# sa2shun/adaptive-speculative-decoding

Hardware: AMD Instinct MI355X
Metric: verified_tokens_per_s (higher is better)
Workload: dtype bf16; 1 GPU; c3: BASELINE headline: batch 32, draft_len 8, vocab 152064 (Qwen2.5), bf16 logits; step = asd_verify_accept_fused_ex: ONE launch (verify + accept + in-kernel stats->MLP->Bayes->DP epilogue); batch_per_gpu=32, draft_len=8, vocab=152064, accumulate=f32 (epilogue f64), rotating_buffers=9, launch_mode=graph, steps_per_graph=2, settle=6000 untimed steps before the 5 warm-up steps (clock / power-state ramp), tiers=7B-draft / 32B / 72B-target shapes (vocab 152064); logits synthetic, parallelism=single GPU

## Files before the change

### adaptive-speculative-decoding_amd/csrc/predictor_device.hpp

```cpp
#pragma once

#include "decision_device.hpp"
#include "lse_device.hpp"

#include <math.h>

#ifndef ASD_EPI_STAMP
#define ASD_EPI_STAMP(slot) do { } while (0)
#endif

namespace asd {

static __device__ double np_sum_leaf(const double* a, int n) {
    if (n < 8) {
        double res = 0.0;
        for (int i = 0; i < n; ++i) res = res + a[i];
        return res;
    }
    double r[8];
#pragma unroll
    for (int j = 0; j < 8; ++j) r[j] = a[j];
    int i = 8;
    for (; i < n - (n % 8); i += 8) {
#pragma unroll
// ... 286 lines not shown
}
__device__ __forceinline__ void decide_and_store_small(const FusedParams& p, int b, float sc, const DecidePrefetch& d) {
    if (p.score) p.score[b] = sc;
    double prob = static_cast<double>(sc);
    if (p.risk) prob = bayes_adjust1(prob, p.n_obs, p.alpha, p.beta);
    if (p.p_hist) {
        p.p_hist[static_cast<int64_t>(b) * p.L + p.stage_idx] = prob;
        if (p.k_star || p.stop) {
            const int n_dp = p.prefix ? p.stage_idx + 1 : p.L;
            double pp[kDecidePrefetch], cc[kDecidePrefetch], J[kDecidePrefetch + 1];
#pragma unroll
            for (int i = 0; i < kDecidePrefetch; ++i) {
                pp[i] = (i == p.stage_idx) ? prob : d.ph[i];
                cc[i] = d.cc[i];
            }
            int ks;
            static_assert(kDecidePrefetch == 4, "the depth switch below lists 1 ... 4");
            (void)J;
            switch (n_dp) {
                case 1: ks = optimal_stopping_exact<1>(pp, cc, p.lam); break;
                case 2: ks = optimal_stopping_exact<2>(pp, cc, p.lam); break;
                case 3: ks = optimal_stopping_exact<3>(pp, cc, p.lam); break;
                default: ks = optimal_stopping_exact<4>(pp, cc, p.lam); break;
            }
            if (p.k_star) p.k_star[b] = ks;
            if (p.stop) p.stop[b] = (ks == p.stage_idx) ? 1 : 0;
        }
    }
    if (p.theta && p.thr_stop) {
        const double q = static_cast<double>(sc);
        p.thr_stop[b] = (q >= d.theta || p.stage_idx == p.L - 1) ? 1 : 0;
    }
}
__device__ __forceinline__ void decide_and_store(const FusedParams& p, int b, float sc) {
    DecidePrefetch none;
    decide_and_store_impl<false>(p, b, sc, none);
}

struct EpiPrefetch {
    float w[32];
    float wd[ASD_NUM_LP_STATS];
    float b1, w2, b2, xv;
    DecidePrefetch d;
};

__device__ __forceinline__ void epi_prefetch(const FusedParams& p, int b, int lane, EpiPrefetch& e) {
    e.xv = p.feat[static_cast<int64_t>(b) * p.ldf + lane];
    const int j = lane & 31, half = lane >> 5;
#pragma unroll
    for (int i = 0; i < 32; ++i) e.w[i] = p.packed[(half * 32 + i) * 32 + j];
#pragma unroll
    for (int d = 0; d < ASD_NUM_LP_STATS; ++d) e.wd[d] = p.stats_col >= 0 ? p.packed[(p.stats_col + d) * 32 + j] : 0.0f;
    e.b1 = p.packed[64 * 32 + j];
    e.w2 = p.packed[64 * 32 + 32 + j];
    e.b2 = p.packed[64 * 32 + 64];
    if (lane == 0) decide_prefetch(p, b, e.d);
}

__device__ __forceinline__ float epi_phase_a_input(const FusedParams& p, int lane, float xv) {
    const int si = lane - p.stats_col;
    return (p.stats_col >= 0 && si >= 0 && si < ASD_NUM_LP_STATS) ? 0.0f : xv;
}
__device__ __forceinline__ float add_halves(float h) {
    const auto r = __builtin_amdgcn_permlane32_swap(__float_as_uint(h), __float_as_uint(h), false, false);
    return __uint_as_float(r[0]) + __uint_as_float(r[1]);
}
template <typename WD>
__device__ __forceinline__ float epi_score(const FusedParams& p, int lane, float h, const WD& wd, const double (&st)[5], bool overlay,
                                           float b1, float w2, float b2) {
    const int half = lane >> 5;
    if (overlay) {
#pragma unroll
        for (int d = 0; d < ASD_NUM_LP_STATS; ++d) {
            const float sd = (half == ((p.stats_col + d) >> 5)) ? static_cast<float>(st[d]) : 0.0f;
            h = fmaf(wd(d), sd, h);
        }
    }
    h = add_halves(h);
    h = fmaxf(h + b1, 0.0f);
    const float z = wave_sum(half == 0 ? w2 * h : 0.0f);
    ASD_EPI_STAMP(10);
    const float e = __builtin_amdgcn_exp2f(-(z + b2) * kLog2e);
    return __builtin_amdgcn_rcpf(1.0f + e);
}

__device__ __forceinline__ void epi_finish(const FusedParams& p, int b, int lane, float lpv, int n, bool want_stats,
                                           const EpiPrefetch& e, double* dvals, float* xs) {
    xs[lane] = epi_phase_a_input(p, lane, e.xv);
    __builtin_amdgcn_fence(__ATOMIC_RELEASE, "wavefront");
    __builtin_amdgcn_wave_barrier();
    __builtin_amdgcn_fence(__ATOMIC_ACQUIRE, "wavefront");
    const int half = lane >> 5;
    float h = 0.0f;
#pragma unroll
    for (int i = 0; i < 32; ++i) h = fmaf(e.w[i], xs[half * 32 + i], h);
    double st[5] = {0.0, 0.0, 0.0, 0.0, 0.0};
    if (want_stats) {
        wave_logprob_stats_regs(lpv, n, lane, st);
        if (p.stats && lane == 0) {
#pragma unroll
            for (int i = 0; i < 5; ++i) p.stats[5 * static_cast<int64_t>(b) + i] = st[i];
        }
    }
    const float sc = epi_score(p, lane, h, [&](int d) { return e.wd[d]; }, st, want_stats && p.stats_col >= 0, e.b1, e.w2, e.b2);
    if (lane == 0) decide_and_store_impl<true>(p, b, sc, e.d);
}


constexpr int kEpiInKernelMaxK = 16;
constexpr int kEpiDecideLds = 12;
__device__ __forceinline__ void epi_decide_dma(const FusedParams& p, int b, int lane, double* dl) {
    typedef __attribute__((address_space(3))) void lds_void;
    typedef const __attribute__((address_space(1))) void glb_void;
    const int n_dp = p.prefix ? p.stage_idx + 1 : p.L;
    if (p.p_hist && (p.k_star || p.stop) && lane < 2 * n_dp) {
        __builtin_amdgcn_global_load_lds((glb_void*)(reinterpret_cast<const char*>(p.p_hist + static_cast<int64_t>(b) * p.L) + lane * 4),
                                         (lds_void*)reinterpret_cast<char*>(dl), 4, 0, 0);
        __builtin_amdgcn_global_load_lds((glb_void*)(reinterpret_cast<const char*>(p.C) + lane * 4),
                                         (lds_void*)(reinterpret_cast<char*>(dl) + 32), 4, 0, 0);
    }
    if (p.theta && p.thr_stop && lane < 2)
        __builtin_amdgcn_global_load_lds((glb_void*)(reinterpret_cast<const char*>(p.theta + p.stage_idx) + lane * 4),
                                         (lds_void*)(reinterpret_cast<char*>(dl) + 64), 4, 0, 0);
}
__device__ __forceinline__ void epi_decide_from_lds(const double* dl, DecidePrefetch& d) {
#pragma unroll
    for (int i = 0; i < kDecidePrefetch; ++i) {
        d.ph[i] = dl[i];
        d.cc[i] = dl[kDecidePrefetch + i];
    }
    d.theta = dl[2 * kDecidePrefetch];
}

struct EpiPhaseA {
    float h, wd[ASD_NUM_LP_STATS], b1, w2, b2;
};
__device__ __forceinline__ void epi_phase_a_lds(const FusedParams& p, int lane, float xv, const float* wl, float* xs, EpiPhaseA& a) {
    xs[lane] = epi_phase_a_input(p, lane, xv);
    __builtin_amdgcn_fence(__ATOMIC_RELEASE, "wavefront");
    __builtin_amdgcn_wave_barrier();
    __builtin_amdgcn_fence(__ATOMIC_ACQUIRE, "wavefront");
    const int j = lane & 31, half = lane >> 5;
    const int col = p.stats_col >= 0 ? p.stats_col : 0;
#pragma unroll
    for (int d = 0; d < ASD_NUM_LP_STATS; ++d) a.wd[d] = wl[(col + d) * 32 + j];
    a.b1 = wl[64 * 32 + j];
    a.w2 = wl[64 * 32 + 32 + j];
    a.b2 = wl[64 * 32 + 64];
    float h = 0.0f;
#pragma unroll
    for (int i = 0; i < 32; ++i) h = fmaf(wl[(half * 32 + i) * 32 + j], xs[half * 32 + i], h);
    a.h = h;
}
__device__ __forceinline__ void epi_finish_lds(const FusedParams& p, int b, int lane, float lpv, int n, bool want_stats,
                                               const double* decide_lds, const EpiPhaseA& a) {
    double st[5] = {0.0, 0.0, 0.0, 0.0, 0.0};
    if (want_stats) {
        wave_logprob_stats_row16(lpv, n, lane, st);
        if (p.stats && lane == 0) {
#pragma unroll
            for (int i = 0; i < 5; ++i) p.stats[5 * static_cast<int64_t>(b) + i] = st[i];
        }
    }
    ASD_EPI_STAMP(9);
    const float sc = epi_score(p, lane, a.h, [&](int d) { return a.wd[d]; }, st, want_stats && p.stats_col >= 0, a.b1, a.w2, a.b2);
    ASD_EPI_STAMP(11);
    if (lane == 0) {
        DecidePrefetch d;
        epi_decide_from_lds(decide_lds, d);
        decide_and_store_small(p, b, sc, d);
    }
}

constexpr int kEpi2In = 256, kEpi2Hid = 128, kEpi2Waves = 8, kEpi2Cols = kEpi2In / kEpi2Waves;
__device__ __forceinline__ void epi2_partial(const float* packed, int w, int lane, float xv, float& h0, float& h1) {
    h0 = 0.0f;
    h1 = 0.0f;
    const float* wp = packed + static_cast<int64_t>(w) * kEpi2Cols * kEpi2Hid + lane;
#pragma unroll 8
    for (int i = 0; i < kEpi2Cols; ++i) {
        const float x = __uint_as_float(__builtin_amdgcn_readlane(__float_as_uint(xv), i));
        h0 = fmaf(wp[i * kEpi2Hid], x, h0);
        h1 = fmaf(wp[i * kEpi2Hid + 64], x, h1);
    }
}
__device__ __forceinline__ float epi2_feature(const float* feat_row, int stats_col, int w, int lane) {
    const int c = w * kEpi2Cols + (lane & 31);
    const float x = feat_row[c];
    const int si = c - stats_col;
    return (stats_col >= 0 && si >= 0 && si < ASD_NUM_LP_STATS) ? 0.0f : x;
}
struct Epi2Tail {
    float wd0[ASD_NUM_LP_STATS], wd1[ASD_NUM_LP_STATS], b1a, b1b, w2a, w2b, b2;
};
__device__ __forceinline__ void epi2_tail_prefetch(const float* packed, int stats_col, int lane, Epi2Tail& t) {
    const int col = stats_col >= 0 ? stats_col : 0;
#pragma unroll
    for (int d = 0; d < ASD_NUM_LP_STATS; ++d) {
        t.wd0[d] = packed[(col + d) * kEpi2Hid + lane];
        t.wd1[d] = packed[(col + d) * kEpi2Hid + 64 + lane];
    }
    const float* b1 = packed + kEpi2In * kEpi2Hid;
    t.b1a = b1[lane]; t.b1b = b1[64 + lane];
    t.w2a = b1[kEpi2Hid + lane]; t.w2b = b1[kEpi2Hid + 64 + lane];
    t.b2 = b1[2 * kEpi2Hid];
}
__device__ __forceinline__ float epi2_score(const float* part, int lane, const Epi2Tail& t, const double (&st)[5], bool overlay) {
    float h0 = part[lane], h1 = part[64 + lane];
#pragma unroll
    for (int w = 1; w < kEpi2Waves; ++w) {
        h0 = h0 + part[w * kEpi2Hid + lane];
        h1 = h1 + part[w * kEpi2Hid + 64 + lane];
    }
    if (overlay) {
#pragma unroll
        for (int d = 0; d < ASD_NUM_LP_STATS; ++d) {
            const float sd = static_cast<float>(st[d]);
            h0 = fmaf(t.wd0[d], sd, h0);
            h1 = fmaf(t.wd1[d], sd, h1);
        }
    }
    h0 = fmaxf(h0 + t.b1a, 0.0f);
    h1 = fmaxf(h1 + t.b1b, 0.0f);
    const float z = wave_sum(fmaf(t.w2b, h1, t.w2a * h0));
    const float e = __builtin_amdgcn_exp2f(-(z + t.b2) * kLog2e);
    return __builtin_amdgcn_rcpf(1.0f + e);
}
__device__ __forceinline__ void epi2_finish_lds(const FusedParams& p, int b, int lane, float lpv, int n, bool want_stats,
                                                const double* decide_lds, const float* part, const Epi2Tail& t) {
    double st[5] = {0.0, 0.0, 0.0, 0.0, 0.0};
    if (want_stats) {
        wave_logprob_stats_row16(lpv, n, lane, st);
        if (p.stats && lane == 0) {
#pragma unroll
            for (int i = 0; i < 5; ++i) p.stats[5 * static_cast<int64_t>(b) + i] = st[i];
        }
    }
    const float sc = epi2_score(part, lane, t, st, want_stats && p.stats_col >= 0);
    if (lane == 0) {
        DecidePrefetch d;
        epi_decide_from_lds(decide_lds, d);
        decide_and_store_small(p, b, sc, d);
    }
}

}
```

### adaptive-speculative-decoding_amd/csrc/verify_accept.hip

```cpp

#include <hip/hip_runtime.h>

#ifdef ASD_STAMP
__device__ unsigned long long* g_asd_stamps = nullptr;
#define ASD_STAMP_AT(slot)                                                                       \
    do {                                                                                         \
        if (threadIdx.x == 0 && g_asd_stamps)                                                    \
            g_asd_stamps[static_cast<size_t>(blockIdx.y * gridDim.x + blockIdx.x) * 16 + (slot)] = __builtin_amdgcn_s_memrealtime(); \
    } while (0)
#define ASD_EPI_STAMP(slot) ASD_STAMP_AT(slot)
#else
#define ASD_STAMP_AT(slot) do { } while (0)
#endif

#define ASD_DPP_ASM_REDUCTIONS 1
#include "lse_device.hpp"
#include "predictor_device.hpp"

namespace asd {
namespace {

constexpr int kMaxStage = 1024;
constexpr int kTicketStride = 160;
constexpr int kLpLineOffset = 32;
constexpr int kSpinLimit = 1 << 20;
constexpr int kFastMaxK = 32;

struct VerifyParams {
    const void* logits;
    int64_t ld_row;
    const int32_t* tok;
    const float* lp_d;
    const float* u;
    int B, K, V, S;
    int64_t v_offset;
    float* lp_t;
    uint8_t* accept;
    int32_t* n_acc;
    uint64_t* bits;
    float* msg;
    uint32_t* tickets;
    uint64_t* granules;
    uint32_t region;
    float scale2;
    int mode;
    float* row_max_lp;
    float* row_entropy;
    int fused;
    int withhold1;
    FusedParams epi;
};

__device__ __forceinline__ uint64_t poll_slot(uint64_t* slot) {
    uint64_t v = __hip_atomic_load(slot, __ATOMIC_RELAXED, __HIP_MEMORY_SCOPE_AGENT);
    for (int spins = 0; v == 0ull && spins < kSpinLimit; ++spins) {
        __builtin_amdgcn_s_sleep(1);
        v = __hip_atomic_load(slot, __ATOMIC_RELAXED, __HIP_MEMORY_SCOPE_AGENT);
    }
    return v;
}

__device__ __forceinline__ uint64_t poll_more(uint64_t* slot, uint64_t v) {
    for (int spins = 0; v == 0ull && spins < kSpinLimit; ++spins) {
        __builtin_amdgcn_s_sleep(1);
        v = __hip_atomic_load(slot, __ATOMIC_RELAXED, __HIP_MEMORY_SCOPE_AGENT);
    }
    return v;
}

__device__ __forceinline__ void report_lost(uint32_t* workspace_words) {
    __hip_atomic_fetch_or(workspace_words, static_cast<uint32_t>(ASD_WS_LOST_HANDOFF), __ATOMIC_RELAXED, __HIP_MEMORY_SCOPE_AGENT);
}

__device__ __forceinline__ void epi_poison(const FusedParams& e, int b) {
    if (e.score) e.score[b] = NAN;
    if (e.k_star) e.k_star[b] = e.L - 1;
    if (e.stop) e.stop[b] = 0;
    if (e.thr_stop) e.thr_stop[b] = 0;
    if (e.stats) {
        for (int i = 0; i < ASD_NUM_LP_STATS; ++i) e.stats[ASD_NUM_LP_STATS * static_cast<int64_t>(b) + i] = NAN;
    }
}

constexpr int kKernargParamsOffset = 48;
static_assert(alignof(VerifyParams) == 8, "kKernargParamsOffset assumes an 8-byte aligned parameter struct");
#define ASD_PIN(x) asm volatile("" : "+s"(x))
template <typename T>
__device__ __forceinline__ T* pin_global_ptr(T* p) {
    uint64_t bits = reinterpret_cast<uint64_t>(p);
    asm volatile("" : "+s"(bits));
    return (T*)(__attribute__((address_space(1))) T*)bits;
}
#define ASD_PIN_PTR(x) do { x = pin_global_ptr(x); } while (0)
__device__ __forceinline__ void pin_epilogue_params(FusedParams& e) {
    ASD_PIN(e.K); ASD_PIN_PTR(e.feat); ASD_PIN(e.ldf); ASD_PIN(e.stats_col); ASD_PIN_PTR(e.packed);
    ASD_PIN(e.risk); ASD_PIN(e.n_obs); ASD_PIN(e.alpha); ASD_PIN(e.beta);
    ASD_PIN_PTR(e.p_hist); ASD_PIN_PTR(e.C); ASD_PIN(e.lam); ASD_PIN(e.L); ASD_PIN(e.stage_idx); ASD_PIN(e.prefix);
    ASD_PIN_PTR(e.theta); ASD_PIN_PTR(e.score); ASD_PIN_PTR(e.k_star); ASD_PIN_PTR(e.stop); ASD_PIN_PTR(e.thr_stop); ASD_PIN_PTR(e.stats);
}

template <int DT, int UNROLL, bool CHECK, bool STATS>
__device__ __forceinline__ void consume(const u32x4 (&r)[UNROLL], uint32_t off, uint32_t end, float c2, float& m2, float& s,
                                        float& t) {
    using E = Elem<DT>;
#pragma unroll
    for (int j = 0; j < UNROLL; ++j) {
        u32x4 v = r[j];
        if (CHECK) {
            const bool ok = off + static_cast<uint32_t>(j) * 1024u < end;
            const u32x4 neg = {E::kNegInfWord, E::kNegInfWord, E::kNegInfWord, E::kNegInfWord};
            v = ok ? v : neg;
        }
        if (STATS) E::accum3(v, c2, m2, s, t);
        else E::accum(v, c2, m2, s);
    }
}

__device__ __forceinline__ float row_max_logprob(float s) {
    return s > 0.0f ? static_cast<float>(-kLn2d * log2_split(s)) : NAN;
}
__device__ __forceinline__ float row_entropy_nats(float m2, float s, float t, float c2) {
    if (!(s > 0.0f)) return NAN;
    const double L = static_cast<double>(m2) + log2_split(s);
    return static_cast<float>(kLn2d * (L - static_cast<double>(c2) * static_cast<double>(t) / static_cast<double>(s)));
}

template <int DT, int THREADS, int UNROLL, bool NT, bool FUSED, bool STATS = false, int EPI = 1>
__global__ __launch_bounds__(THREADS) void k_verify(const void* a_logits, const int32_t* a_tok, int64_t a_ld_row, int a_V,
                                                    int a_K, int a_S, float a_scale2, int a_own, const VerifyParams p) {
    using E = Elem<DT>;
    constexpr int kWaves = THREADS / 64;
    __shared__ uint32_t next_tile;
    __shared__ __attribute__((aligned(16))) uint64_t stage[kMaxStage];
    __shared__ float stage_t[STATS ? kMaxStage : 1];
    static_assert(EPI == 1 || (EPI == 2 && THREADS == 64 * kEpi2Waves), "the 256 x 128 epilogue is cut over eight waves");
    __shared__ __attribute__((aligned(16))) float wlds[FUSED ? (EPI == 2 ? kEpi2Waves * kEpi2Hid : 64 * 32 + 68) : 4];
    __shared__ __attribute__((aligned(16))) double dlds[FUSED ? kEpiDecideLds : 1];

    ASD_STAMP_AT(0);
#ifdef ASD_STAMP
    if (threadIdx.x == 0 && g_asd_stamps)
        g_asd_stamps[static_cast<size_t>(blockIdx.y * gridDim.x + blockIdx.x) * 16 + 6] = __builtin_amdgcn_s_getreg((31 << 11) | 20) & 0xf;
#endif
    const int tid = threadIdx.x;
    const int lane = tid & 63;
    const int wave = tid >> 6;
    const int S = a_S;
    const float c2 = a_scale2;
    const int row = static_cast<int>(blockIdx.x);
    const int split = static_cast<int>(blockIdx.y);

    const char* rowp = static_cast<const char*>(a_logits) + static_cast<int64_t>(row) * a_ld_row * E::kBytes;
    const uint32_t mis = static_cast<uint32_t>(reinterpret_cast<uintptr_t>(rowp) & 15u);
    int head = mis ? static_cast<int>((16u - mis) / E::kBytes) : 0;
    if (head > a_V) head = a_V;
    const int nvec = (a_V - head) / E::kPerVec;
    const int tail = a_V - head - nvec * E::kPerVec;
    const char* body = rowp + static_cast<int64_t>(head) * E::kBytes;
    int v0 = 0, v1 = nvec;
    if (S > 1) {
        v0 = static_cast<int>(static_cast<uint32_t>(nvec) * static_cast<uint32_t>(split) / static_cast<uint32_t>(S));
        v1 = static_cast<int>(static_cast<uint32_t>(nvec) * static_cast<uint32_t>(split + 1) / static_cast<uint32_t>(S));
    }

    const bool own_row = a_own != 0;
    float x_tok = -INFINITY, lpd = 0.0f, uu = 1.0f;
    uint32_t raw_tok = 0, raw_lpd = 0, raw_u = 0x3f800000u, raw_x = 0;
    bool have_x = false;
    double lu_row = 0.0;
    int vrow = row;
    asm volatile("" : "+v"(vrow));
    const bool gather = own_row || split == 0;
    if (gather && tid == 0) raw_tok = static_cast<uint32_t>(a_tok[vrow]);

    constexpr uint32_t kTileBytes = static_cast<uint32_t>(UNROLL) * 1024u;
    const uint32_t end = v1 > v0 ? static_cast<uint32_t>(v1 - v0) * 16u : 0u;
    const uint32_t n_tiles = (end + kTileBytes - 1) / kTileBytes;
    const uint32_t n_full = end / kTileBytes;
    const __amdgpu_buffer_rsrc_t rsrc = __builtin_amdgcn_make_buffer_rsrc(
        const_cast<char*>(body) + static_cast<int64_t>(v0) * 16, 0, static_cast<int>(end), 0x00020000);
    const uint32_t lane_off = static_cast<uint32_t>(lane) * 16u;
    if (tid == 0) next_tile = 2u * kWaves;
    uint32_t ta = static_cast<uint32_t>(wave), tb = static_cast<uint32_t>(wave) + kWaves;
    u32x4 ra[UNROLL], rb[UNROLL];
#pragma unroll
    for (int j = 0; j < UNROLL; ++j) ra[j] = load16<NT>(rsrc, ta * kTileBytes + static_cast<uint32_t>(j) * 1024u + lane_off);
#pragma unroll
    for (int j = 0; j < UNROLL; ++j) rb[j] = load16<NT>(rsrc, tb * kTileBytes + static_cast<uint32_t>(j) * 1024u + lane_off);
    ASD_STAMP_AT(7);
    __syncthreads();

    asm volatile("" : "+v"(raw_tok));
    const int64_t t_tok = static_cast<int64_t>(static_cast<int32_t>(raw_tok)) - p.v_offset;
    if (gather && tid == 0 && t_tok >= 0 && t_tok < a_V) {
        raw_x = E::raw(rowp, t_tok);
        have_x = true;
    }
    if (own_row && tid == 0 && p.mode == 0) {
        raw_lpd = reinterpret_cast<const uint32_t*>(p.lp_d)[vrow];
        raw_u = reinterpret_cast<const uint32_t*>(p.u)[vrow];
    }
    uint32_t raw_head = 0, raw_tail = 0, raw_feat = 0;
    const bool do_head = wave == 0 && split == 0 && lane < head;
    const bool do_tail = wave == 0 && split == S - 1 && lane >= 32 && lane - 32 < tail;
    if (do_head) raw_head = E::raw(rowp, lane);
    if (do_tail) raw_tail = E::raw(rowp, static_cast<int64_t>(head) + static_cast<int64_t>(nvec) * E::kPerVec + (lane - 32));
    const int b = static_cast<int>(static_cast<uint32_t>(row) / static_cast<uint32_t>(a_K));
    const int k = row - b * a_K;
    const bool fused = FUSED && p.mode == 0;
#define ASD_CLAIM(dst)                                                                                   \
    do {                                                                                                 \
        uint32_t c_ = 0;                                                                                 \
        if (lane == 0) c_ = __hip_atomic_fetch_add(&next_tile, 1u, __ATOMIC_RELAXED, __HIP_MEMORY_SCOPE_WORKGROUP); \
        dst = __builtin_amdgcn_readfirstlane(c_);                                                        \
    } while (0)
#define ASD_REDUCE_TILE(reg, t)                                                                          \
    do {                                                                                                 \
        float tm_ = kSentinel, ts_ = 0.0f, tt_ = 0.0f;                                                   \
        if ((t) < n_full) consume<DT, UNROLL, false, STATS>(reg, (t) * kTileBytes + lane_off, end, c2, tm_, ts_, tt_);   \
        else consume<DT, UNROLL, true, STATS>(reg, (t) * kTileBytes + lane_off, end, c2, tm_, ts_, tt_);                 \
        if (STATS) wave_merge3(tm_, ts_, tt_);                                                           \
        else wave_merge(tm_, ts_);                                                                       \
        if (lane == 0) {                                                                                 \
            stage[(t)] = (static_cast<uint64_t>(__float_as_uint(ts_)) << 32) | __float_as_uint(tm_);     \
            if (STATS) stage_t[(t)] = tt_;                                                               \
        }                                                                                                \
    } while (0)

    bool first = true;
    while (ta < n_tiles) {
        uint32_t tn;
        ASD_CLAIM(tn);
        ASD_REDUCE_TILE(ra, ta);
        if (first) { ASD_STAMP_AT(1); first = false; }
        ta = tn;
#if defined(ASD_LAB) && ASD_LAB == 10
#pragma unroll
        for (int j = 0; j < UNROLL; ++j) asm volatile("" : "+v"(ra[j]));
#else
#pragma unroll
        for (int j = 0; j < UNROLL; ++j) ra[j] = load16<NT>(rsrc, ta * kTileBytes + static_cast<uint32_t>(j) * 1024u + lane_off);
#endif
        if (tb >= n_tiles) break;
        ASD_CLAIM(tn);
        ASD_REDUCE_TILE(rb, tb);
        tb = tn;
#if defined(ASD_LAB) && ASD_LAB == 10
#pragma unroll
        for (int j = 0; j < UNROLL; ++j) asm volatile("" : "+v"(rb[j]));
#else
#pragma unroll
        for (int j = 0; j < UNROLL; ++j) rb[j] = load16<NT>(rsrc, tb * kTileBytes + static_cast<uint32_t>(j) * 1024u + lane_off);
#endif
    }
#undef ASD_CLAIM
#undef ASD_REDUCE_TILE

    ASD_STAMP_AT(2);
#ifdef ASD_STAMP
    if (lane == 0 && g_asd_stamps)
        g_asd_stamps[static_cast<size_t>(gridDim.x * gridDim.y) * 16 + static_cast<size_t>(blockIdx.y * gridDim.x + blockIdx.x) * 16 + wave] = __builtin_amdgcn_s_memrealtime();
#endif
#if defined(ASD_LAB) && (ASD_LAB == 8 || ASD_LAB == 10)
    if (lane == 0 && stage[0] == 0x1234567812345678ull) p.lp_t[row] = 0.0f;
    return;
#endif
    FusedParams ep;
    const int wave_u = __builtin_amdgcn_readfirstlane(wave);
    const bool fin_wg = FUSED && fused && k == a_K - 1 && (own_row || split == S - 1);
    float xv2 = 0.0f;
    const float* packed2 = nullptr;
    int col2 = -1;
    if constexpr (FUSED && EPI == 2) {
        if (fin_wg) {
            typedef const __attribute__((address_space(4))) char* ka_ptr2;
            typedef const __attribute__((address_space(4))) FusedParams* ka_epi_ptr2;
            ka_ptr2 ka2 = (ka_ptr2)__builtin_amdgcn_kernarg_segment_ptr();
            asm volatile("" : "+s"(ka2));
            const ka_epi_ptr2 kp2 = (ka_epi_ptr2)(ka2 + kKernargParamsOffset + __builtin_offsetof(VerifyParams, epi));
            const float* feat2 = pin_global_ptr(kp2->feat);
            int64_t ldf2 = kp2->ldf;
            col2 = kp2->stats_col;
            packed2 = pin_global_ptr(kp2->packed);
            ASD_PIN(ldf2); ASD_PIN(col2);
            xv2 = epi2_feature(feat2 + static_cast<int64_t>(b) * ldf2, col2, wave_u, lane);
        }
    }
    if (wave_u == 0) {
        asm volatile("" : "+v"(raw_x), "+v"(raw_head), "+v"(raw_tail), "+v"(raw_lpd), "+v"(raw_u));
        if (FUSED) {
            typedef const __attribute__((address_space(4))) char* ka_ptr;
            typedef const __attribute__((address_space(4))) FusedParams* ka_epi_ptr;
            ka_ptr ka = (ka_ptr)__builtin_amdgcn_kernarg_segment_ptr();
            asm volatile("" : "+s"(ka));
            const ka_epi_ptr kp = (ka_epi_ptr)(ka + kKernargParamsOffset + __builtin_offsetof(VerifyParams, epi));
            ep.lp = nullptr; ep.ld_lp = 0; ep.n_valid = nullptr; ep.in_dim = 64; ep.hidden = 32; ep.use_lds = 0; ep.B = 0;
            ep.K = kp->K; ep.feat = kp->feat; ep.ldf = kp->ldf; ep.stats_col = kp->stats_col; ep.packed = kp->packed;
            ep.risk = kp->risk; ep.n_obs = kp->n_obs; ep.alpha = kp->alpha; ep.beta = kp->beta;
            ep.p_hist = kp->p_hist; ep.C = kp->C; ep.lam = kp->lam; ep.L = kp->L; ep.stage_idx = kp->stage_idx; ep.prefix = kp->prefix;
            ep.theta = kp->theta; ep.score = kp->score; ep.k_star = kp->k_star; ep.stop = kp->stop; ep.thr_stop = kp->thr_stop;
            ep.stats = kp->stats;
            pin_epilogue_params(ep);
#if defined(ASD_LAB) && ASD_LAB == 5
            if (false) {
#else
            if (EPI == 1 && fin_wg) {
#endif
                typedef __attribute__((address_space(3))) void lds_void;
                typedef const __attribute__((address_space(1))) void glb_void;
                const char* src = reinterpret_cast<const char*>(ep.packed);
#pragma unroll
                for (int ps = 0; ps < 8; ++ps)
                    __builtin_amdgcn_global_load_lds((glb_void*)(src + ps * 1024 + lane * 16), (lds_void*)(reinterpret_cast<char*>(wlds) + ps * 1024), 16, 0, 0);
                __builtin_amdgcn_global_load_lds((glb_void*)(src + 8192 + lane * 4), (lds_void*)(reinterpret_cast<char*>(wlds) + 8192), 4, 0, 0);
                if (lane == 0)
                    __builtin_amdgcn_global_load_lds((glb_void*)(src + 8192 + 256), (lds_void*)(reinterpret_cast<char*>(wlds) + 8192 + 256), 4, 0, 0);
                raw_feat = reinterpret_cast<const uint32_t*>(ep.feat)[static_cast<int64_t>(b) * ep.ldf + lane];
            }
        }
        float hm = kSentinel, hs = 0.0f, ht = 0.0f;
        if (do_head) {
            const float xv = E::from_raw(raw_head);
            accum_scalar(xv, c2, hm, hs);
            if (STATS) ht = hs > 0.0f ? hs * xv : 0.0f;
        }
        if (do_tail) {
            const float xv = E::from_raw(raw_tail);
            accum_scalar(xv, c2, hm, hs);
            if (STATS) ht = hs > 0.0f ? hs * xv : 0.0f;
        }
        if (STATS) wave_merge3(hm, hs, ht);
        else wave_merge(hm, hs);
        if (lane == 0) {
            stage[n_tiles] = (static_cast<uint64_t>(__float_as_uint(hs)) << 32) | __float_as_uint(hm);
            if (STATS) stage_t[n_tiles] = ht;
        }
        if (gather && tid == 0) {
            if (have_x) x_tok = E::from_raw(raw_x);
            if (own_row && p.mode == 0) {
                lpd = __uint_as_float(raw_lpd);
                uu = __uint_as_float(raw_u);
                lu_row = log_u(uu);
            }
        }
    }
    __syncthreads();
    if (wave_u != 0) {
        if constexpr (FUSED && EPI == 2) {
            if (fin_wg) {
                float h0, h1;
                epi2_partial(packed2, wave_u, lane, xv2, h0, h1);
                wlds[wave_u * kEpi2Hid + lane] = h0;
                wlds[wave_u * kEpi2Hid + 64 + lane] = h1;
                __syncthreads();
            }
        }
        return;
    }
    float m2 = kSentinel, s = 0.0f, tsum = 0.0f;
    for (uint32_t t = static_cast<uint32_t>(lane); t <= n_tiles; t += 64) {
        const uint64_t g = stage[t];
        if (STATS) ms_merge3(m2, s, tsum, __uint_as_float(static_cast<uint32_t>(g)), __uint_as_float(static_cast<uint32_t>(g >> 32)), stage_t[t]);
        else ms_merge(m2, s, __uint_as_float(static_cast<uint32_t>(g)), __uint_as_float(static_cast<uint32_t>(g >> 32)));
    }
    if (STATS) wave_merge3(m2, s, tsum);
    else wave_merge(m2, s);
    __builtin_amdgcn_fence(__ATOMIC_RELEASE, "wavefront");
    __builtin_amdgcn_wave_barrier();
    ASD_STAMP_AT(3);

    if (own_row) {
        if (!(FUSED && fused) && lane != 0) return;
        if (p.mode == 1) {
            p.msg[3 * row + 0] = m2;
            p.msg[3 * row + 1] = s;
            p.msg[3 * row + 2] = x_tok;
            return;
        }
        uint32_t* line = p.tickets + static_cast<int64_t>(b) * kTicketStride;
        if (FUSED && fused) {
            float lp = 0.0f;
            bool flag = false;
            if (lane == 0) flag = finish_row(m2, s, x_tok, c2, lpd, lu_row, lp);
            uint64_t* slots = reinterpret_cast<uint64_t*>(line + kLpLineOffset);
            const uint64_t mine = (1ull << 63) | (static_cast<uint64_t>(flag ? 1u : 0u) << 32) | __float_as_uint(lp);
            if (k != p.K - 1) {
                if (lane == 0) {
                    if (row + 1 != p.withhold1) __hip_atomic_store(slots + k, mine, __ATOMIC_RELAXED, __HIP_MEMORY_SCOPE_AGENT);
                    p.lp_t[row] = lp;
                    p.accept[row] = flag ? 1 : 0;
                    if (p.row_max_lp) p.row_max_lp[row] = row_max_logprob(s);
                }
                return;
            }
            ASD_STAMP_AT(4);
            uint64_t sv = __shfl(mine, 0, 64);
            EpiPhaseA pa{};
            Epi2Tail tail2{};
            if constexpr (EPI == 1) {
                asm volatile("s_waitcnt vmcnt(0)" : "+v"(raw_feat) :: "memory");
                if (lane < p.K - 1) sv = __hip_atomic_load(slots + lane, __ATOMIC_RELAXED, __HIP_MEMORY_SCOPE_AGENT);
                epi_phase_a_lds(ep, lane, __uint_as_float(raw_feat), wlds, reinterpret_cast<float*>(stage + 192), pa);
                uint32_t sv_lo = static_cast<uint32_t>(sv), sv_hi = static_cast<uint32_t>(sv >> 32);
                asm volatile("" : "+v"(pa.h), "+v"(pa.wd[0]), "+v"(pa.wd[1]), "+v"(pa.wd[2]), "+v"(pa.wd[3]), "+v"(pa.wd[4]), "+v"(pa.b1), "+v"(pa.w2),
                             "+v"(pa.b2), "+v"(sv_lo), "+v"(sv_hi));
                sv = (static_cast<uint64_t>(sv_hi) << 32) | sv_lo;
            } else {
                if (lane < p.K - 1) sv = __hip_atomic_load(slots + lane, __ATOMIC_RELAXED, __HIP_MEMORY_SCOPE_AGENT);
                epi2_tail_prefetch(packed2, col2, lane, tail2);
                float h0, h1;
                epi2_partial(packed2, 0, lane, xv2, h0, h1);
                wlds[lane] = h0;
                wlds[64 + lane] = h1;
                __syncthreads();
                uint32_t sv_lo = static_cast<uint32_t>(sv), sv_hi = static_cast<uint32_t>(sv >> 32);
                asm volatile("" : "+v"(sv_lo), "+v"(sv_hi));
                sv = (static_cast<uint64_t>(sv_hi) << 32) | sv_lo;
            }
            epi_decide_dma(ep, b, lane, dlds);
            if (lane == 0) {
                p.lp_t[row] = lp;
                p.accept[row] = flag ? 1 : 0;
                if (p.row_max_lp) p.row_max_lp[row] = row_max_logprob(s);
            }
#if defined(ASD_LAB) && (ASD_LAB == 2 || ASD_LAB == 5)
            sv = __shfl(mine, 0, 64);
            if (lane < p.K - 1) __hip_atomic_store(slots + lane, 0ull, __ATOMIC_RELAXED, __HIP_MEMORY_SCOPE_AGENT);
#else
            if (lane < p.K - 1) {
                sv = poll_more(slots + lane, sv);
                __hip_atomic_store(slots + lane, 0ull, __ATOMIC_RELAXED, __HIP_MEMORY_SCOPE_AGENT);
            }
#endif
            const bool lost = lane < p.K && sv == 0ull;
            const unsigned long long bal = __ballot(lane < p.K && ((sv >> 32) & 1ull));
            if (lane == 0) {
                const unsigned long long inv = ~bal;
                const int n = inv ? __builtin_ctzll(inv) : 64;
                p.n_acc[b] = n < p.K ? n : p.K;
                if (p.bits) p.bits[b] = bal;
            }
            ASD_STAMP_AT(5);
            if (__ballot(lost) != 0ull) {
                if (lane == 0) {
                    epi_poison(ep, b);
                    report_lost(p.tickets);
                }
                return;
            }
#if defined(ASD_LAB) && (ASD_LAB == 1 || ASD_LAB == 2 || ASD_LAB == 5)
            if (lane == 0 && ep.score) ep.score[b] = pa.h + pa.wd[0] + pa.b1 + pa.w2 + pa.b2 + __uint_as_float(static_cast<uint32_t>(sv));
            return;
#endif
            if constexpr (EPI == 1)
                epi_finish_lds(ep, b, lane, __uint_as_float(static_cast<uint32_t>(sv)), p.K, ep.stats_col >= 0 || ep.stats != nullptr, dlds, pa);
            else
                epi2_finish_lds(ep, b, lane, __uint_as_float(static_cast<uint32_t>(sv)), p.K, ep.stats_col >= 0 || ep.stats != nullptr, dlds, wlds, tail2);
            ASD_STAMP_AT(8);
            return;
        }
        if (lane == 0) {
            float lp;
            const bool flag = finish_row(m2, s, x_tok, c2, lpd, lu_row, lp);
            p.lp_t[row] = lp;
            p.accept[row] = flag ? 1 : 0;
            if (p.row_max_lp) p.row_max_lp[row] = row_max_logprob(s);
            if (STATS) {
                if (p.row_entropy) p.row_entropy[row] = row_entropy_nats(m2, s, tsum, c2);
            }
            uint64_t* word = reinterpret_cast<uint64_t*>(line + 2);
            const uint64_t mine = (1ull << 32) | (static_cast<uint64_t>(flag ? 1u : 0u) << k);
            ASD_STAMP_AT(4);
#if defined(ASD_LAB) && ASD_LAB == 9
            if (mine == 0x1234ull) p.n_acc[b] = 0;
            return;
#endif
            const uint64_t old = __hip_atomic_fetch_add(word, mine, __ATOMIC_RELAXED, __HIP_MEMORY_SCOPE_AGENT);
            if (static_cast<uint32_t>(old >> 32) == static_cast<uint32_t>(p.K - 1)) {
                const uint32_t mask = static_cast<uint32_t>(old | mine);
                const uint32_t inv = ~mask;
                const int n = inv ? __builtin_ctz(inv) : 32;
                p.n_acc[b] = n < p.K ? n : p.K;
                if (p.bits) p.bits[b] = mask;
                __hip_atomic_store(word, 0ull, __ATOMIC_RELAXED, __HIP_MEMORY_SCOPE_AGENT);
            }
#ifdef ASD_STAMP
            asm volatile("s_waitcnt vmcnt(0)" ::: "memory");
            if (g_asd_stamps) g_asd_stamps[static_cast<size_t>(blockIdx.y * gridDim.x + blockIdx.x) * 16 + 5] = __builtin_amdgcn_s_memrealtime() + (old & 0);
#endif
        }
        return;
    }

    const int KS = p.K * S;
    uint64_t* region = p.granules + static_cast<int64_t>(b) * p.region;
    uint64_t* xslots = reinterpret_cast<uint64_t*>(p.tickets + static_cast<int64_t>(b) * kTicketStride + kLpLineOffset);
    if (lane == 0 && row * S + split + 1 != p.withhold1) {
        const uint64_t g = (static_cast<uint64_t>(__float_as_uint(s)) << 32) | __float_as_uint(m2);
        __hip_atomic_store(region + k * S + split, g, __ATOMIC_RELAXED, __HIP_MEMORY_SCOPE_AGENT);
        if (split == 0)
            __hip_atomic_store(xslots + k, (1ull << 63) | __float_as_uint(x_tok), __ATOMIC_RELAXED, __HIP_MEMORY_SCOPE_AGENT);
    }
    if (k != p.K - 1 || split != S - 1) return;

    const int frow = b * p.K + lane;
    if (FUSED) {
        if (fused) asm volatile("s_waitcnt vmcnt(0)" : "+v"(raw_feat) :: "memory");
    }
    uint64_t xv0 = 0ull, gv0 = 0ull;
    if (lane < p.K) {
        if (p.mode == 0) { lpd = p.lp_d[frow]; uu = p.u[frow]; }
        xv0 = __hip_atomic_load(xslots + lane, __ATOMIC_RELAXED, __HIP_MEMORY_SCOPE_AGENT);
    }
    if (lane < KS) gv0 = __hip_atomic_load(region + lane, __ATOMIC_RELAXED, __HIP_MEMORY_SCOPE_AGENT);
    EpiPhaseA pa{};
    if constexpr (FUSED && EPI == 1) {
        if (fused) {
            epi_phase_a_lds(ep, lane, __uint_as_float(raw_feat), wlds, reinterpret_cast<float*>(stage + 192), pa);
            uint32_t a0 = static_cast<uint32_t>(xv0), a1 = static_cast<uint32_t>(xv0 >> 32), g0 = static_cast<uint32_t>(gv0), g1 = static_cast<uint32_t>(gv0 >> 32);
            asm volatile("" : "+v"(pa.h), "+v"(pa.wd[0]), "+v"(pa.wd[1]), "+v"(pa.wd[2]), "+v"(pa.wd[3]), "+v"(pa.wd[4]), "+v"(pa.b1), "+v"(pa.w2), "+v"(pa.b2),
                         "+v"(a0), "+v"(a1), "+v"(g0), "+v"(g1));
            xv0 = (static_cast<uint64_t>(a1) << 32) | a0;
            gv0 = (static_cast<uint64_t>(g1) << 32) | g0;
            epi_decide_dma(ep, b, lane, dlds);
            __builtin_amdgcn_fence(__ATOMIC_RELEASE, "wavefront");
            __builtin_amdgcn_wave_barrier();
        }
    }
    bool lost_x = false;
    if (lane < p.K) {
        const uint64_t xv = poll_more(xslots + lane, xv0);
        __hip_atomic_store(xslots + lane, 0ull, __ATOMIC_RELAXED, __HIP_MEMORY_SCOPE_AGENT);
        lost_x = xv == 0ull;
        x_tok = __uint_as_float(static_cast<uint32_t>(xv));
    }
    for (int g = lane; g < KS; g += 64) {
        stage[g] = g == lane ? poll_more(region + g, gv0) : poll_slot(region + g);
        __hip_atomic_store(region + g, 0ull, __ATOMIC_RELAXED, __HIP_MEMORY_SCOPE_AGENT);
    }
    __builtin_amdgcn_fence(__ATOMIC_RELEASE, "wavefront");
    __builtin_amdgcn_wave_barrier();
    __builtin_amdgcn_fence(__ATOMIC_ACQUIRE, "wavefront");

    float fm = kSentinel, fs = 0.0f;
    bool lost = lost_x;
    if (lane < p.K) {
#pragma unroll 4
        for (int j = 0; j < S; ++j) {
            const uint64_t g = stage[lane * S + j];
            lost = lost || g == 0ull;
            ms_merge(fm, fs, __uint_as_float(static_cast<uint32_t>(g)), __uint_as_float(static_cast<uint32_t>(g >> 32)));
        }
        if (lost) { fm = NAN; fs = NAN; }
    }
    if (__ballot(lost) != 0ull && lane == 0) report_lost(p.tickets);

    if (p.mode == 1) {
        if (lane < p.K) {
            p.msg[3 * frow + 0] = fm;
            p.msg[3 * frow + 1] = fs;
            p.msg[3 * frow + 2] = x_tok;
        }
        return;
    }
    bool flag = false;
    float lp = 0.0f;
    if (lane < p.K) {
        flag = finish_row(fm, fs, x_tok, c2, lpd, log_u(uu), lp);
        p.lp_t[frow] = lp;
        p.accept[frow] = flag ? 1 : 0;
        if (p.row_max_lp) p.row_max_lp[frow] = row_max_logprob(fs);
    }
    finish_sequence(flag, lane, p.K, b, p.n_acc, p.bits);
    if constexpr (FUSED && EPI == 1) {
        if (!fused) return;
        if (__ballot(lost) != 0ull) {
            if (lane == 0) epi_poison(ep, b);
            return;
        }
        epi_finish_lds(ep, b, lane, lp, p.K, ep.stats_col >= 0 || ep.stats != nullptr, dlds, pa);
        ASD_STAMP_AT(8);
    }
}

__global__ __launch_bounds__(64) void k_accept_from_partials(const float* msg_all, int n_shards, const float* lp_d,
                                                             const float* u, int B, int K, float c2, float* lp_t,
// ... 380 lines not shown
```

Measured before the change: 10.51 million tokens/s.

## Split fused epilogue tail across helper waves for weight load, MLP and ticket polling

In the workgroup that owns the final row, two otherwise idle waves now run the epilogue preparation in parallel with wave 0's verify work. One wave DMAs the MLP weights into LDS and computes the hidden layer. The other loads the decision tables, polls the ticket slots and clears them. Wave 0 syncs with them through __syncthreads and reads the precomputed hidden activations and slot values from new LDS buffers, so it no longer does this serial work itself. The cost is extra barriers, extra LDS, and a tighter coupling between waves that could deadlock or stall if the barrier counts ever differ between paths.

```diff
diff --git a/adaptive-speculative-decoding_amd/csrc/predictor_device.hpp b/adaptive-speculative-decoding_amd/csrc/predictor_device.hpp
--- a/adaptive-speculative-decoding_amd/csrc/predictor_device.hpp
+++ b/adaptive-speculative-decoding_amd/csrc/predictor_device.hpp
@@ -462,6 +462,16 @@
     for (int i = 0; i < 32; ++i) h = fmaf(wl[(half * 32 + i) * 32 + j], xs[half * 32 + i], h);
     a.h = h;
 }
+__device__ __forceinline__ void epi_phase_a_from_lds(const FusedParams& p, int lane, const float* wl, const float* hs, EpiPhaseA& a) {
+    const int j = lane & 31;
+    const int col = p.stats_col >= 0 ? p.stats_col : 0;
+#pragma unroll
+    for (int d = 0; d < ASD_NUM_LP_STATS; ++d) a.wd[d] = wl[(col + d) * 32 + j];
+    a.b1 = wl[64 * 32 + j];
+    a.w2 = wl[64 * 32 + 32 + j];
+    a.b2 = wl[64 * 32 + 64];
+    a.h = hs[lane];
+}
 __device__ __forceinline__ void epi_finish_lds(const FusedParams& p, int b, int lane, float lpv, int n, bool want_stats,
                                                const double* decide_lds, const EpiPhaseA& a) {
     double st[5] = {0.0, 0.0, 0.0, 0.0, 0.0};
diff --git a/adaptive-speculative-decoding_amd/csrc/verify_accept.hip b/adaptive-speculative-decoding_amd/csrc/verify_accept.hip
--- a/adaptive-speculative-decoding_amd/csrc/verify_accept.hip
+++ b/adaptive-speculative-decoding_amd/csrc/verify_accept.hip
@@ -9,8 +9,14 @@
             g_asd_stamps[static_cast<size_t>(blockIdx.y * gridDim.x + blockIdx.x) * 16 + (slot)] = __builtin_amdgcn_s_memrealtime(); \
     } while (0)
 #define ASD_EPI_STAMP(slot) ASD_STAMP_AT(slot)
+#define ASD_STAMP_WAVE(slot)                                                                     \
+    do {                                                                                         \
+        if ((threadIdx.x & 63) == 0 && g_asd_stamps)                                             \
+            g_asd_stamps[static_cast<size_t>(blockIdx.y * gridDim.x + blockIdx.x) * 16 + (slot)] = __builtin_amdgcn_s_memrealtime(); \
+    } while (0)
 #else
 #define ASD_STAMP_AT(slot) do { } while (0)
+#define ASD_STAMP_WAVE(slot) do { } while (0)
 #endif
 
 #define ASD_DPP_ASM_REDUCTIONS 1
@@ -82,8 +88,12 @@
     }
 }
 
-constexpr int kKernargParamsOffset = 48;
-static_assert(alignof(VerifyParams) == 8, "kKernargParamsOffset assumes an 8-byte aligned parameter struct");
+struct VerifyKernargs {
+    const void* a_logits; const int32_t* a_tok; int64_t a_ld_row; int a_V, a_K, a_S; float a_scale2; int a_own;
+    VerifyParams p;
+};
+constexpr int kKernargParamsOffset = static_cast<int>(__builtin_offsetof(VerifyKernargs, p));
+static_assert(kKernargParamsOffset == 48 && alignof(VerifyParams) == 8, "k_verify's by-value parameter struct starts at byte 48 of its kernarg segment");
 #define ASD_PIN(x) asm volatile("" : "+s"(x))
 template <typename T>
 __device__ __forceinline__ T* pin_global_ptr(T* p) {
@@ -97,6 +107,18 @@
     ASD_PIN(e.risk); ASD_PIN(e.n_obs); ASD_PIN(e.alpha); ASD_PIN(e.beta);
     ASD_PIN_PTR(e.p_hist); ASD_PIN_PTR(e.C); ASD_PIN(e.lam); ASD_PIN(e.L); ASD_PIN(e.stage_idx); ASD_PIN(e.prefix);
     ASD_PIN_PTR(e.theta); ASD_PIN_PTR(e.score); ASD_PIN_PTR(e.k_star); ASD_PIN_PTR(e.stop); ASD_PIN_PTR(e.thr_stop); ASD_PIN_PTR(e.stats);
+}
+
+__device__ __forceinline__ void epi_weights_dma(const float* packed, float* wl, int lane) {
+    typedef __attribute__((address_space(3))) void lds_void;
+    typedef const __attribute__((address_space(1))) void glb_void;
+    const char* src = reinterpret_cast<const char*>(packed);
+#pragma unroll
+    for (int ps = 0; ps < 8; ++ps)
+        __builtin_amdgcn_global_load_lds((glb_void*)(src + ps * 1024 + lane * 16), (lds_void*)(reinterpret_cast<char*>(wl) + ps * 1024), 16, 0, 0);
+    __builtin_amdgcn_global_load_lds((glb_void*)(src + 8192 + lane * 4), (lds_void*)(reinterpret_cast<char*>(wl) + 8192), 4, 0, 0);
+    if (lane == 0)
+        __builtin_amdgcn_global_load_lds((glb_void*)(src + 8192 + 256), (lds_void*)(reinterpret_cast<char*>(wl) + 8192 + 256), 4, 0, 0);
 }
 
 template <int DT, int UNROLL, bool CHECK, bool STATS>
@@ -136,6 +158,11 @@
     static_assert(EPI == 1 || (EPI == 2 && THREADS == 64 * kEpi2Waves), "the 256 x 128 epilogue is cut over eight waves");
     __shared__ __attribute__((aligned(16))) float wlds[FUSED ? (EPI == 2 ? kEpi2Waves * kEpi2Hid : 64 * 32 + 68) : 4];
     __shared__ __attribute__((aligned(16))) double dlds[FUSED ? kEpiDecideLds : 1];
+    constexpr bool kTail3 = FUSED && EPI == 1;
+    __shared__ __attribute__((aligned(16))) float tail_f[kTail3 ? 128 : 1];
+    __shared__ __attribute__((aligned(16))) uint64_t tail_slots[kTail3 ? kEpiInKernelMaxK : 1];
+    static_assert(!kTail3 || sizeof(stage) + sizeof(wlds) + sizeof(dlds) + sizeof(tail_f) + sizeof(tail_slots) + 16 <= 18 * 1024,
+                  "LDS of the one-launch instantiation");
 
     ASD_STAMP_AT(0);
 #ifdef ASD_STAMP
@@ -286,6 +313,59 @@
             xv2 = epi2_feature(feat2 + static_cast<int64_t>(b) * ldf2, col2, wave_u, lane);
         }
     }
+    const bool tail3 = FUSED && EPI == 1 && fin_wg && own_row;
+    if constexpr (FUSED && EPI == 1) {
+        if (tail3 && (wave_u == 1 || wave_u == 2)) {
+            typedef const __attribute__((address_space(4))) char* ka_ptr1;
+            typedef const __attribute__((address_space(4))) FusedParams* ka_epi_ptr1;
+            ka_ptr1 ka1 = (ka_ptr1)__builtin_amdgcn_kernarg_segment_ptr();
+            asm volatile("" : "+s"(ka1));
+            const ka_epi_ptr1 kp1 = (ka_epi_ptr1)(ka1 + kKernargParamsOffset + __builtin_offsetof(VerifyParams, epi));
+            if (wave_u == 1) {
+                FusedParams ep1{};
+                const float* packed1 = kp1->packed;
+                const float* feat1 = kp1->feat;
+                int64_t ldf1 = kp1->ldf;
+                ep1.stats_col = kp1->stats_col;
+                ASD_PIN_PTR(packed1); ASD_PIN_PTR(feat1); ASD_PIN(ldf1); ASD_PIN(ep1.stats_col);
+#if !(defined(ASD_LAB) && ASD_LAB == 5)
+                epi_weights_dma(packed1, wlds, lane);
+                raw_feat = reinterpret_cast<const uint32_t*>(feat1)[static_cast<int64_t>(b) * ldf1 + lane];
+#endif
+                __syncthreads();
+                asm volatile("s_waitcnt vmcnt(0)" : "+v"(raw_feat) :: "memory");
+                EpiPhaseA pa1;
+                epi_phase_a_lds(ep1, lane, __uint_as_float(raw_feat), wlds, tail_f, pa1);
+                tail_f[64 + lane] = pa1.h;
+                ASD_STAMP_WAVE(12);
+                __syncthreads();
+            } else {
+                FusedParams ep2{};
+                typedef uint32_t* const __attribute__((address_space(4)))* ka_tickets_ptr;
+                uint32_t* tickets2 = *(ka_tickets_ptr)(ka1 + kKernargParamsOffset + __builtin_offsetof(VerifyParams, tickets));
+                ep2.p_hist = kp1->p_hist; ep2.C = kp1->C; ep2.L = kp1->L; ep2.stage_idx = kp1->stage_idx; ep2.prefix = kp1->prefix;
+                ep2.theta = kp1->theta; ep2.k_star = kp1->k_star; ep2.stop = kp1->stop; ep2.thr_stop = kp1->thr_stop;
+                ASD_PIN_PTR(tickets2); ASD_PIN_PTR(ep2.p_hist); ASD_PIN_PTR(ep2.C); ASD_PIN(ep2.L); ASD_PIN(ep2.stage_idx); ASD_PIN(ep2.prefix);
+                ASD_PIN_PTR(ep2.theta); ASD_PIN_PTR(ep2.k_star); ASD_PIN_PTR(ep2.stop); ASD_PIN_PTR(ep2.thr_stop);
+                __syncthreads();
+                uint64_t* slots2 = reinterpret_cast<uint64_t*>(tickets2 + static_cast<int64_t>(b) * kTicketStride + kLpLineOffset);
+                uint64_t sv2 = 0ull;
+#if defined(ASD_LAB) && (ASD_LAB == 2 || ASD_LAB == 5)
+                epi_decide_dma(ep2, b, lane, dlds);
+#else
+                if (lane < a_K - 1) sv2 = __hip_atomic_load(slots2 + lane, __ATOMIC_RELAXED, __HIP_MEMORY_SCOPE_AGENT);
+                epi_decide_dma(ep2, b, lane, dlds);
+                if (lane < a_K - 1) sv2 = poll_more(slots2 + lane, sv2);
+#endif
+                asm volatile("s_waitcnt vmcnt(0)" ::: "memory");
+                if (lane < kEpiInKernelMaxK) tail_slots[lane] = sv2;
+                ASD_STAMP_WAVE(13);
+                __syncthreads();
+                if (lane < a_K - 1) __hip_atomic_store(slots2 + lane, 0ull, __ATOMIC_RELAXED, __HIP_MEMORY_SCOPE_AGENT);
+            }
+            return;
+        }
+    }
     if (wave_u == 0) {
         asm volatile("" : "+v"(raw_x), "+v"(raw_head), "+v"(raw_tail), "+v"(raw_lpd), "+v"(raw_u));
         if (FUSED) {
@@ -304,17 +384,9 @@
 #if defined(ASD_LAB) && ASD_LAB == 5
             if (false) {
 #else
-            if (EPI == 1 && fin_wg) {
-#endif
-                typedef __attribute__((address_space(3))) void lds_void;
-                typedef const __attribute__((address_space(1))) void glb_void;
-                const char* src = reinterpret_cast<const char*>(ep.packed);
-#pragma unroll
-                for (int ps = 0; ps < 8; ++ps)
-                    __builtin_amdgcn_global_load_lds((glb_void*)(src + ps * 1024 + lane * 16), (lds_void*)(reinterpret_cast<char*>(wlds) + ps * 1024), 16, 0, 0);
-                __builtin_amdgcn_global_load_lds((glb_void*)(src + 8192 + lane * 4), (lds_void*)(reinterpret_cast<char*>(wlds) + 8192), 4, 0, 0);
-                if (lane == 0)
-                    __builtin_amdgcn_global_load_lds((glb_void*)(src + 8192 + 256), (lds_void*)(reinterpret_cast<char*>(wlds) + 8192 + 256), 4, 0, 0);
+            if (EPI == 1 && fin_wg && !own_row) {
+#endif
+                epi_weights_dma(ep.packed, wlds, lane);
                 raw_feat = reinterpret_cast<const uint32_t*>(ep.feat)[static_cast<int64_t>(b) * ep.ldf + lane];
             }
         }
@@ -394,18 +466,24 @@
                 return;
             }
             ASD_STAMP_AT(4);
-            uint64_t sv = __shfl(mine, 0, 64);
+            uint64_t sv;
             EpiPhaseA pa{};
             Epi2Tail tail2{};
             if constexpr (EPI == 1) {
-                asm volatile("s_waitcnt vmcnt(0)" : "+v"(raw_feat) :: "memory");
-                if (lane < p.K - 1) sv = __hip_atomic_load(slots + lane, __ATOMIC_RELAXED, __HIP_MEMORY_SCOPE_AGENT);
-                epi_phase_a_lds(ep, lane, __uint_as_float(raw_feat), wlds, reinterpret_cast<float*>(stage + 192), pa);
-                uint32_t sv_lo = static_cast<uint32_t>(sv), sv_hi = static_cast<uint32_t>(sv >> 32);
-                asm volatile("" : "+v"(pa.h), "+v"(pa.wd[0]), "+v"(pa.wd[1]), "+v"(pa.wd[2]), "+v"(pa.wd[3]), "+v"(pa.wd[4]), "+v"(pa.b1), "+v"(pa.w2),
-                             "+v"(pa.b2), "+v"(sv_lo), "+v"(sv_hi));
-                sv = (static_cast<uint64_t>(sv_hi) << 32) | sv_lo;
+                if (lane == 0) {
+                    p.lp_t[row] = lp;
+                    p.accept[row] = flag ? 1 : 0;
+                    if (p.row_max_lp) p.row_max_lp[row] = row_max_logprob(s);
+                }
+                __syncthreads();
+                sv = (static_cast<uint64_t>(__builtin_amdgcn_readfirstlane(static_cast<uint32_t>(mine >> 32))) << 32) |
+                     __builtin_amdgcn_readfirstlane(static_cast<uint32_t>(mine));
+#if !(defined(ASD_LAB) && (ASD_LAB == 2 || ASD_LAB == 5))
+                if (lane < p.K - 1) sv = tail_slots[lane];
+#endif
+                epi_phase_a_from_lds(ep, lane, wlds, tail_f + 64, pa);
             } else {
+                sv = __shfl(mine, 0, 64);
                 if (lane < p.K - 1) sv = __hip_atomic_load(slots + lane, __ATOMIC_RELAXED, __HIP_MEMORY_SCOPE_AGENT);
                 epi2_tail_prefetch(packed2, col2, lane, tail2);
                 float h0, h1;
@@ -417,6 +495,7 @@
                 asm volatile("" : "+v"(sv_lo), "+v"(sv_hi));
                 sv = (static_cast<uint64_t>(sv_hi) << 32) | sv_lo;
             }
+            if constexpr (EPI != 1) {
             epi_decide_dma(ep, b, lane, dlds);
             if (lane == 0) {
                 p.lp_t[row] = lp;
@@ -432,6 +511,7 @@
                 __hip_atomic_store(slots + lane, 0ull, __ATOMIC_RELAXED, __HIP_MEMORY_SCOPE_AGENT);
             }
 #endif
+            }
             const bool lost = lane < p.K && sv == 0ull;
             const unsigned long long bal = __ballot(lane < p.K && ((sv >> 32) & 1ull));
             if (lane == 0) {
```

Result: no change. 10.57 million tokens/s (median of 5 runs) (+0.6%).
